# drowe67/radae

Measured on AMD Instinct MI355X. Metric: vocoder-feature frames/sec (enc+chan+dec), model19, higher is better.
Workload: dtype f32 I/O, 2xf16 (22-bit) MFMA operands, f32 accumulate (refine: f64 MFMA)

## Files before the change

radae_amd/csrc/rade_dev.h:

```cpp
#ifndef RADE_DEV_H
#define RADE_DEV_H

#include <stdint.h>

#ifdef __cplusplus
extern "C" {
#endif

#define RD_M        160
#define RD_NCP      32
#define RD_SYM      192
#define RD_NC       30
#define RD_NS       4
#define RD_NMF      960
#define RD_NEOO     1152
#define RD_RXBUF    2112
#define RD_NFC      40
#define RD_NQ       16
#define RD_NTAP     101
#define RD_NINMAX   1120
#define RD_LATENT   80
#define RD_ZMF      240
#define RD_FEAT_MF  432
#define RD_NEOOBITS 180
// ... 61 lines not shown
    int uw_errors, synced_count, snr_int, pad;
    double fmax, Dthresh, Dtmax12, Dtmax12_eoo;
    float snrdB_3k_est; float pad2;
} rd_rx_trace;

typedef void *rd_stream_t;

typedef struct {
    const float *a1; long a1_sb, a1_st; int K1;
    const float *a0; long a0_sb, a0_st; int K0;
    const int *reset; int reset_sb;
    const int *n_rows;
    const float *Wp; const float *bias;
    const unsigned short *Wp16;
    const float *Wscale;
    float *y; long y_sb, y_st; int N;
    int B, T, act;
} rd_gemm_args;
int rd_launch_gemm(const rd_gemm_args *a, rd_stream_t s);
long rd_pack_weights(const float *W, int N, int K, float *out);
long rd_packed_size(int N, int K);

typedef struct {
    const float *gi; long gi_sb, gi_st;
    const float *Whh; const float *bhh;
    float *h;
    float *out; long out_sb, out_st;
    const int *reset; int reset_sb;
    const int *n_rows;
    int B, T, H;
    unsigned short *outf; int outf_NQ, outf_col;
} rd_scan_args;
int rd_launch_gru_scan(const rd_scan_args *a, rd_stream_t s);

#define RD_EF_KB   (RD_ENC_W / 16)
#define RD_EF_TILE (RD_EF_KB * 1024)
typedef struct {
    const unsigned short *xf; int NQ;
    int B, T, K0, K1, dil;
    const unsigned short *Wp16; const float *Wscale; const float *bias; int N, act;
    float *y; long y_sb, y_st;
    unsigned short *yf; int ycol;
    int seq_taps, no_pair;
    int pair;
    const float *xin; int Kin; const float *Wp;
} rd_encf_args;
int rd_launch_encf_gemm(const rd_encf_args *a, rd_stream_t s);
int rd_launch_encf_dense1(const rd_encf_args *a, rd_stream_t s);
int rd_launch_encf_hist(unsigned short *xf, int NQ, float *x32, long x32_sb, int B, int T, int dir, rd_stream_t s);

int rd_launch_enc_pack(const float *features, float *xin, int B, int T, rd_stream_t s);
int rd_launch_pad_rows(const float *src, float *dst, long R, int K, int Kpad, rd_stream_t s);
int rd_launch_chan_symbol(const float *z, const float *H, const float *noise, float *out, long n_real, int mode, float p0, float p1, unsigned long long seed, rd_stream_t s);
int rd_launch_carry_rows(float *x, int B, int Tcap, int W, int nhist, int T, const int *n_rows, rd_stream_t s);
int rd_launch_ofdm_mod(const rd_tables *tab, const float *z, void *tx, long tx_stride, int B, int n_mf, int linear, rd_stream_t s);
int rd_launch_ofdm_mod_mp(const rd_tables *tab, const float *z, void *tx, long tx_stride, int B, int n_mf, const void *G, void *mp, double *part, int linear, rd_stream_t s);
int rd_launch_eoo_build(const rd_tables *tab, const float *bits, float *eoo, int B, rd_stream_t s);
int rd_launch_copy_eoo(const float *eoo, void *out, long stride, int B, rd_stream_t s);

enum { RD_IRX_LS = 0, RD_IRX_MEAN6 = 1, RD_IRX_ALL = 2, RD_IRX_NONE = 3 };
typedef struct {
    const rd_tables *tab; const void *rx; long rx_stride;
    const float *foff;
    int n_mf, time_offset, eq, coarse_mag, B;
    float mag_scale;
    float *z_hat;
// ... 142 lines not shown
```

radae_amd/csrc/rade_devutil.h:

```cpp
#ifndef RADE_DEVUTIL_H
#define RADE_DEVUTIL_H
#include <hip/hip_runtime.h>
#include <stdint.h>
#include <math.h>

#include "rade_dev.h"

typedef float f32x16 __attribute__((ext_vector_type(16)));
typedef float f32x4 __attribute__((ext_vector_type(4)));
typedef float f32x2 __attribute__((ext_vector_type(2)));
typedef unsigned u32x4 __attribute__((ext_vector_type(4)));
__device__ __forceinline__ f32x2 pk_fma(f32x2 a, f32x2 b, f32x2 c) { return __builtin_elementwise_fma(a, b, c); }
typedef double f64x4 __attribute__((ext_vector_type(4)));
typedef _Float16 f16x8 __attribute__((ext_vector_type(8)));

#define PI_D 3.14159265358979323846

__device__ __forceinline__ float2 cmul(float2 a, float2 b) { return make_float2(a.x * b.x - a.y * b.y, a.x * b.y + a.y * b.x); }
__device__ __forceinline__ float2 cmul_nc(float2 a, float2 b)
{
#pragma clang fp contract(off)
    const float rr = a.x * b.x, ii = a.y * b.y, ri = a.x * b.y, ir = a.y * b.x;
    return make_float2(rr - ii, ri + ir);
}
// ... 17 lines not shown
    acc[0] = fmaf(sy.y, -w.y, acc[0]); acc[1] = fmaf(sy.y, w.x, acc[1]);
    return acc;
}

__device__ __forceinline__ float2 cadd(float2 a, float2 b) { return make_float2(a.x + b.x, a.y + b.y); }
__device__ __forceinline__ double chan_phase_acc(int i, float f0, float df_dt)
{
    if (df_dt == 0.0f) { const float om = ((f0 * 2.0f) * (float)PI_D) / 8000.0f; return (double)(i + 1) * (double)om; }
    const double n = (double)(i + 1);
    return (2.0 * PI_D / 8000.0) * (n * (double)f0 + ((double)df_dt / 8000.0) * 0.5 * (double)i * n);
}
__device__ __forceinline__ float2 cconj(float2 a) { return make_float2(a.x, -a.y); }
__device__ __forceinline__ float2 unit_conj(float2 c)
{
    const float n2 = c.x * c.x + c.y * c.y;
    if (n2 == 0.0f) return make_float2(1.0f, 0.0f);
    const float inv = 1.0f / sqrtf(n2);
    return make_float2(c.x * inv, -c.y * inv);
}
__device__ __forceinline__ float2 cis_reduced(double ang)
{
    const double r = ang - 6.283185307179586476925 * rint(ang * 0.15915494309189533577);
    float sn, cs; sincosf((float)r, &sn, &cs);
    return make_float2(cs, sn);
}
__device__ __forceinline__ float sigmoid_f(float x) { return 1.0f / (1.0f + expf(-x)); }
__device__ __forceinline__ int rx_tid() { int t = threadIdx.x; asm volatile("" : "+v"(t)); return t; }
template <int CTRL> __device__ __forceinline__ float quad_dpp(float x) { return __int_as_float(__builtin_amdgcn_update_dpp(0, __float_as_int(x), CTRL, 0xF, 0xF, true)); }
#define QUAD_XOR1 0xB1
#define QUAD_XOR2 0x4E
#define QUAD_BC0  0x00
#define QUAD_BC1  0x55
#define QUAD_BC2  0xAA
#define ROW_ROR4  0x124
#define ROW_ROR8  0x128
template <int CTRL> __device__ __forceinline__ int quad_dpp_i(int x) { return __builtin_amdgcn_update_dpp(0, x, CTRL, 0xF, 0xF, true); }
template <int CTRL> __device__ __forceinline__ double dpp_f64(double x)
{
    const long long b = __double_as_longlong(x);
    const unsigned lo = (unsigned)quad_dpp_i<CTRL>((int)(unsigned)b), hi = (unsigned)quad_dpp_i<CTRL>((int)(unsigned)(b >> 32));
    return __longlong_as_double((long long)(((unsigned long long)hi << 32) | lo));
}
__device__ __forceinline__ double wave_sum_f64(double v)
{
    v += dpp_f64<QUAD_XOR1>(v); v += dpp_f64<QUAD_XOR2>(v); v += dpp_f64<ROW_ROR4>(v); v += dpp_f64<ROW_ROR8>(v);
    const long long b = __double_as_longlong(v);
    double t = 0.0;
#pragma unroll
    for (int r = 0; r < 4; r++) {
        const unsigned lo = (unsigned)__builtin_amdgcn_readlane((int)(unsigned)b, 16 * r), hi = (unsigned)__builtin_amdgcn_readlane((int)(unsigned)(b >> 32), 16 * r);
        t += __longlong_as_double((long long)(((unsigned long long)hi << 32) | lo));
    }
    return t;
}
__device__ __forceinline__ float wave_sum_f32(float v)
{
    v += quad_dpp<QUAD_XOR1>(v); v += quad_dpp<QUAD_XOR2>(v); v += quad_dpp<ROW_ROR4>(v); v += quad_dpp<ROW_ROR8>(v);
    float t = 0.0f;
#pragma unroll
    for (int r = 0; r < 4; r++) t += __int_as_float(__builtin_amdgcn_readlane(__float_as_int(v), 16 * r));
    return t;
}
__device__ __forceinline__ float wave_max_f32(float v)
{
    v = fmaxf(v, quad_dpp<QUAD_XOR1>(v)); v = fmaxf(v, quad_dpp<QUAD_XOR2>(v)); v = fmaxf(v, quad_dpp<ROW_ROR4>(v)); v = fmaxf(v, quad_dpp<ROW_ROR8>(v));
    float t = 0.0f;
// ... 51 lines not shown
```

radae_amd/csrc/rade_engine.c:

```c
#define _GNU_SOURCE
#define __HIP_PLATFORM_AMD__ 1
#include <hip/hip_runtime_api.h>

#include <pthread.h>
#include <time.h>
#include <sched.h>
#include <stdio.h>
#include <stdlib.h>
#include <string.h>
#include <stdint.h>
#include <math.h>

#include "rade_batch.h"
#include "rade_api.h"
#include "rade_host.h"

#define CHK(x) do { hipError_t e_ = (x); if (e_ != hipSuccess) { fprintf(stderr, "rade: HIP error %s at %s:%d\n", hipGetErrorString(e_), __FILE__, __LINE__); goto fail; } } while (0)

static int g_engines_open;
double rade_host_cpu_quota(void)
{
    cpu_set_t set; double n = 1.0;
    if (sched_getaffinity(0, sizeof set, &set) == 0) n = (double)CPU_COUNT(&set);
    FILE *f = fopen("/sys/fs/cgroup/cpu.max", "r");
// ... 9 lines not shown
static pthread_once_t g_sync_once = PTHREAD_ONCE_INIT;
static void sync_policy_init(void)
{
    const char *e = getenv("RADE_SYNC"), *p = getenv("RADE_SYNC_PEERS");
    g_sync_quota = rade_host_cpu_quota(); g_sync_peers = p && atoi(p) > 1 ? atoi(p) : 1;
    g_sync_mode = e && !strcmp(e, "block") ? 1 : (e && !strcmp(e, "spin") ? 0 : 2);
}
static int sync_blocking_now(void)
{
    pthread_once(&g_sync_once, sync_policy_init);
    return g_sync_mode == 2 ? rade_sync_policy(__atomic_load_n(&g_engines_open, __ATOMIC_RELAXED) * g_sync_peers, g_sync_quota) : g_sync_mode;
}

typedef struct { float *wp, *bias; unsigned short *wp16, *wa16; float *wscale, *wscale16; int N, K; } dev_lin;

#define ON_DEV(h) do { if (h) (void)hipSetDevice((h)->device); } while (0)

#define RADE_PROF_MAXEV 256
#define RADE_PROF_MAXIV 4096
struct rade_batch {
    struct owned *owned;
    int alloc_failed;
    int B, max_tx_mf, device, flags, trace_cap, Tcap;
    int R, dec_rows;
    int unsync_off_after;
    unsigned short *corrq16, *corra16, *wfwd16, *bpf16; double *vm; int rx_lds, rx_census;
    int feat_in, enc_kpad, bottleneck1;
    float *dec2_x, *dec2_gi, *dec2_hbuf, *dec2_h[5];
    rd_tables *d_tab;
    dev_lin enc_dense1, enc_zdense, dec_dense1, dec_output, enc_gin[5], dec_gin[5], enc_conv[5], dec_conv[5], dec_glu[5];
    float *enc_whh[5], *enc_bhh[5], *dec_whh[5], *dec_bhh[5];
    unsigned short *dec_whq[5]; float *dec_whs[5];
    float *enc_xin, *enc_x, *enc_gi, *enc_h[5], *enc_z, *eoo, *eoo_bits;
    unsigned short *enc_xf; int enc_nq, enc_seq_taps, enc_no_pair;
    int enc_hist_frag;
    int bypass_dec;
    int tx_linear;
    double *irx_part; long irx_part_cap; float *irx_foff; long long *irx_err;
    rd_bpf_state *tx_bpf, *tx_bpf_init; void *tx_raw; float *tx_chain; float *eoo_filt;
    void *chan_scratch; void *chan_mp;
    float *chan_ps, *chan_ps_host;
    float *rs_sigma; double *rs_part, *rs_stats;
    float *clk_taps; rd_clk_stream *clk_ps, *clk_ps_host;
    int *loss_len; double *loss_res, *loss_part; long loss_part_cap;
    rd_rx_stream *rx_st; rd_rx_round *rx_round;
    int *rx_avail, *rx_acc, *rx_progress, *rx_status;
    float *zrows, *dec_x, *dec_gi, *dec_hbuf, *dec_h[5], *feat84, *dtcache;
    void *rx_filt; float *bpf_chain; long filt_cap, chain_stride;
    rd_rx_trace *trace; float *trace_z;
    long long *wg_cycles;
    int *h_small;
    unsigned *lcg_seeds;
    unsigned *d_lcg_seeds;
    int prof_on, prof_cnt; hipEvent_t prof_ev[2 * RADE_PROF_MAXEV]; int prof_cls[RADE_PROF_MAXEV]; double prof_fl[RADE_PROF_MAXEV];
    double prof_ms[RADE_PROF_NCLASS], prof_flops[RADE_PROF_NCLASS]; long prof_n[RADE_PROF_NCLASS];
    hipEvent_t prof_ref; int iv_n; int iv_cls[RADE_PROF_MAXIV]; float iv_t0[RADE_PROF_MAXIV], iv_t1[RADE_PROF_MAXIV];
    hipEvent_t ev_block;
    long n_sync_block, n_sync_spin;
    double wait_est_us;
};

static const int ENC_IN[5] = { 64, 224, 384, 544, 704 };
static const int ENC_DIL[5] = { 1, 2, 2, 2, 2 };
static const int DEC_IN[5] = { 96, 224, 352, 480, 608 };
static long tx_raw_stride(const rade_batch *h) { return (long)(h->max_tx_mf > 2 ? h->max_tx_mf : 2) * RD_NMF; }

struct owned { struct owned *next; void *p; int pinned; };
// ... 181 lines not shown
    if (h->alloc_failed || h->rx_lds <= 0) goto fail;

    int err = 0;
    h->feat_in = m.enc_dense1.n_in; h->enc_kpad = (h->feat_in + 15) & ~15; h->bottleneck1 = (cfg->flags & RADE_BATCH_BOTTLENECK1) != 0;
    err |= upload_lin(h, &h->enc_dense1, m.enc_dense1.w, m.enc_dense1.b, NULL, 64, h->feat_in, h->enc_kpad);
    err |= upload_lin(h, &h->enc_zdense, m.enc_zdense.w, m.enc_zdense.b, NULL, 80, 864, 864);
    err |= upload_lin(h, &h->dec_dense1, m.dec_dense1.w, m.dec_dense1.b, NULL, 96, 80, 80);
    err |= upload_lin(h, &h->dec_output, m.dec_output.w, m.dec_output.b, NULL, h->feat_in, 736, 736);
    for (int l = 0; l < 5 && !err; l++) {
        err |= upload_lin(h, &h->enc_gin[l], m.enc_gru[l].w_ih, m.enc_gru[l].b_ih, m.enc_gru[l].s_ih, 192, ENC_IN[l], ENC_IN[l]);
        err |= upload_lin(h, &h->dec_gin[l], m.dec_gru[l].w_ih, m.dec_gru[l].b_ih, m.dec_gru[l].s_ih, 288, DEC_IN[l], DEC_IN[l]);
        err |= upload_lin(h, &h->enc_conv[l], m.enc_conv[l].w, m.enc_conv[l].b, m.enc_conv[l].row_scale, 96, m.enc_conv[l].n_in, m.enc_conv[l].n_in);
        err |= upload_lin(h, &h->dec_conv[l], m.dec_conv[l].w, m.dec_conv[l].b, m.dec_conv[l].row_scale, 32, m.dec_conv[l].n_in, m.dec_conv[l].n_in);
        err |= upload_lin(h, &h->dec_glu[l], m.dec_glu[l].w, NULL, m.dec_glu[l].row_scale, 96, 96, 96);
        h->enc_whh[l] = dev_upload(h, m.enc_gru[l].w_hh, sizeof(float) * 192 * 64);
        h->enc_bhh[l] = dev_upload(h, m.enc_gru[l].b_hh, sizeof(float) * 192);
        h->dec_whh[l] = dev_upload(h, m.dec_gru[l].w_hh, sizeof(float) * 288 * 96);
        h->dec_bhh[l] = dev_upload(h, m.dec_gru[l].b_hh, sizeof(float) * 288);
        if (m.dec_gru[l].s_hh) {
            unsigned short *pa = malloc(sizeof(unsigned short) * rd_packed16a_size(288, 96)); float *scl = malloc(sizeof(float) * 288);
            const long nq = (pa && scl) ? rd_pack_weights_q16_a16(m.dec_gru[l].w_hh, m.dec_gru[l].s_hh, 288, 96, pa, scl) : -1;
            if (nq > 0) { h->dec_whq[l] = dev_upload_opt(h, pa, sizeof(unsigned short) * nq); h->dec_whs[l] = dev_upload_opt(h, scl, sizeof(float) * 288); }
            free(pa); free(scl);
        }
    }
    if (err || h->alloc_failed) { fprintf(stderr, "rade: weight upload failed\n"); goto fail; }

    h->enc_xin = dev_zeros(h, sizeof(float) * B * T * RD_ENC_IN);
    h->enc_x = dev_zeros(h, sizeof(float) * B * (2 + T) * RD_ENC_W);
    h->enc_gi = dev_zeros(h, sizeof(float) * B * T * 192);
    h->enc_nq = 1 + (h->Tcap + 31) / 32;
    h->enc_seq_taps = getenv("RADE_ENCF_SEQ_TAPS") != NULL;
    h->enc_no_pair = getenv("RADE_ENCF_NO_PAIR") != NULL;
    if (B * T > 16384 && !getenv("RADE_ENC_ROWS")) {
        h->enc_xf = dev_alloc_opt(h, sizeof(unsigned short) * B * h->enc_nq * RD_EF_TILE, 1);
        if (!h->enc_xf && !getenv("RADE_VERBOSE_0"))
            fprintf(stderr, "rade: no device memory for the encoder's fragment buffer (%.1f MB): the float32-row kernels serve every call (slower encoder GEMMs, same results to the last bits documented in rade_batch.h)\n",
                    1e-6 * sizeof(unsigned short) * (double)B * h->enc_nq * RD_EF_TILE);
    }
    h->enc_z = dev_zeros(h, sizeof(float) * B * T * RD_LATENT);
    h->eoo = dev_zeros(h, sizeof(float) * B * RD_NEOO * 2);
    h->eoo_bits = dev_zeros(h, sizeof(float) * B * RD_NEOOBITS);
    h->bypass_dec = (cfg->flags & RADE_BATCH_BYPASS_DEC) != 0;
    h->tx_linear = (cfg->flags & RADE_BATCH_TX_LINEAR) != 0;
    if (h->tx_linear && (cfg->flags & RADE_BATCH_TX_BPF)) { fprintf(stderr, "rade: RADE_BATCH_TX_LINEAR cannot be combined with RADE_BATCH_TX_BPF (the filter clips)\n"); goto fail; }
    if (cfg->flags & RADE_BATCH_TX_BPF) {
        rd_bpf_state *init = calloc(B, sizeof *init);
        if (!init) goto fail;
        for (size_t b = 0; b < B; b++) { init[b].mem_len = 100; init[b].phase[0] = 1.0f; }
        h->tx_bpf_init = dev_upload(h, init, sizeof(rd_bpf_state) * B); h->tx_bpf = dev_upload(h, init, sizeof(rd_bpf_state) * B);
        free(init);
        h->tx_raw = dev_zeros(h, sizeof(float) * 2 * B * tx_raw_stride(h));
        h->tx_chain = dev_zeros(h, sizeof(float) * 2 * B * (cfg->max_tx_mf + 8));
        h->eoo_filt = dev_zeros(h, sizeof(float) * 2 * B * RD_NEOO);
    }
    h->chan_scratch = dev_zeros(h, sizeof(double) * B * (1 + (cfg->max_tx_mf > 64 ? cfg->max_tx_mf : 64)) * 2);
    h->enc_h[0] = dev_zeros(h, sizeof(float) * 5 * B * 64); h->dec_h[0] = dev_zeros(h, sizeof(float) * 5 * B * 96);
    h->dec2_h[0] = dev_zeros(h, sizeof(float) * 5 * B * 96);
    h->rx_progress = dev_zeros(h, sizeof(int) * (8 + B * 8));
    if (h->alloc_failed) { fprintf(stderr, "rade: device allocation failed\n"); goto fail; }
    for (int l = 1; l < 5; l++) { h->enc_h[l] = h->enc_h[0] + (size_t)l * B * 64; h->dec_h[l] = h->dec_h[0] + (size_t)l * B * 96; }
    for (int l = 1; l < 5; l++) h->dec2_h[l] = h->dec2_h[0] + (size_t)l * B * 96;
    h->rx_acc = h->rx_progress + 8; h->rx_status = h->rx_progress + 8 + 4 * B;
    h->rx_st = dev_zeros(h, sizeof(rd_rx_stream) * B);
    h->rx_round = dev_zeros(h, sizeof(rd_rx_round) * B);
    h->rx_avail = dev_zeros(h, sizeof(int) * B);
// ... 116 lines not shown
    PROF_END(hh, stream, RADE_PROF_GEMM, 2.0 * (double)B * T * (K0 + K1) * w->N);
    return rc;
}

static int encf_gemm(rade_batch *h, const dev_lin *w, int K1, int K0, int dil, float *y, long y_sb, long y_st, int ycol, int T, int act, void *stream)
{
    rd_encf_args g;
    memset(&g, 0, sizeof g);
    g.xf = h->enc_xf; g.NQ = h->enc_nq; g.B = h->B; g.T = T; g.K0 = K0; g.K1 = K1; g.dil = dil;
    g.Wp16 = w->wp16; g.Wscale = w->wscale16; g.bias = w->bias; g.N = w->N; g.act = act;
    g.y = y; g.y_sb = y_sb; g.y_st = y_st; if (!y) { g.yf = h->enc_xf; g.ycol = ycol; }
    g.seq_taps = h->enc_seq_taps; g.no_pair = h->enc_no_pair;
    if (K0 + K1 != w->K || !w->wp16) { fprintf(stderr, "rade: internal GEMM shape error (%d+%d != %d)\n", K0, K1, w->K); return -1; }
    PROF_BEGIN(h, stream);
    const int rc = rd_launch_encf_gemm(&g, stream);
    PROF_END(h, stream, RADE_PROF_GEMM, 2.0 * (double)h->B * T * (K0 + K1) * w->N);
    return rc;
}
static int encode_core_frag(rade_batch *h, int T, float *z, void *stream)
{
    const int B = h->B;
    int e = h->enc_hist_frag ? 0 : rd_launch_encf_hist(h->enc_xf, h->enc_nq, h->enc_x, (long)(2 + h->Tcap) * RD_ENC_W, B, T, 0, stream);
    {
        rd_encf_args g;
        memset(&g, 0, sizeof g);
        g.xf = h->enc_xf; g.NQ = h->enc_nq; g.B = B; g.T = T; g.bias = h->enc_dense1.bias; g.N = 64; g.act = 1; g.yf = h->enc_xf; g.ycol = 0;
        g.xin = h->enc_xin; g.Kin = h->enc_kpad; g.Wp = h->enc_dense1.wp;
        PROF_BEGIN(h, stream); e |= rd_launch_encf_dense1(&g, stream); PROF_END(h, stream, RADE_PROF_GEMM, 2.0 * (double)B * T * h->enc_kpad * 64);
    }
    e |= encf_gemm(h, &h->enc_gin[0], ENC_IN[0], 0, 0, h->enc_gi, (long)T * 192, 192, 0, T, 0, stream);
    for (int l = 0; l < 5 && !e; l++) {
        const int in = ENC_IN[l], cin = in + 64;
        rd_scan_args s = { h->enc_gi, (long)T * 192, 192, h->enc_whh[l], h->enc_bhh[l], h->enc_h[l], NULL, 0, 0, NULL, 0, NULL, B, T, 64, h->enc_xf, h->enc_nq, in };
        PROF_BEGIN(h, stream); e |= rd_launch_gru_scan(&s, stream); PROF_END(h, stream, RADE_PROF_SCAN, 2.0 * B * T * 192 * 64);
        e |= encf_gemm(h, &h->enc_conv[l], cin, cin, ENC_DIL[l], NULL, 0, 0, cin, T, 1, stream);
        if (l < 4) e |= encf_gemm(h, &h->enc_gin[l + 1], ENC_IN[l + 1], 0, 0, h->enc_gi, (long)T * 192, 192, 0, T, 0, stream);
        else e |= encf_gemm(h, &h->enc_zdense, 864, 0, 0, z, (long)T * RD_LATENT, RD_LATENT, 0, T, h->bottleneck1 ? 1 : 0, stream);
    }
    e |= rd_launch_encf_hist(h->enc_xf, h->enc_nq, h->enc_x, (long)(2 + h->Tcap) * RD_ENC_W, B, T, 1, stream);
    h->enc_hist_frag = !e;
    return e;
}

static int encode_core(rade_batch *h, int T, float *z, void *stream)
{
    const int B = h->B, W = RD_ENC_W;
    if (h->enc_xf && (long)B * T > 16384) return encode_core_frag(h, T, z, stream);
    h->enc_hist_frag = 0;
    const long xsb = (long)(2 + h->Tcap) * W;
    float *x0 = h->enc_x + 2 * W;
    int e = 0;
    dev_lin d1 = h->enc_dense1; d1.wp16 = NULL; d1.wscale16 = NULL;
    e |= gemm(h, &d1, h->enc_xin, (long)T * h->enc_kpad, h->enc_kpad, h->enc_kpad, NULL, 0, 0, 0, NULL, NULL, x0, xsb, W, B, T, 1, stream);
    for (int l = 0; l < 5 && !e; l++) {
        const int in = ENC_IN[l], cin = in + 64;
        e |= gemm(h, &h->enc_gin[l], x0, xsb, W, in, NULL, 0, 0, 0, NULL, NULL, h->enc_gi, (long)T * 192, 192, B, T, 0, stream);
        rd_scan_args s = { h->enc_gi, (long)T * 192, 192, h->enc_whh[l], h->enc_bhh[l], h->enc_h[l], x0 + in, xsb, W, NULL, 0, NULL, B, T, 64 };
        PROF_BEGIN(h, stream); e |= rd_launch_gru_scan(&s, stream); PROF_END(h, stream, RADE_PROF_SCAN, 2.0 * B * T * 192 * 64);
        e |= gemm(h, &h->enc_conv[l], x0, xsb, W, cin, x0 - (long)ENC_DIL[l] * W, xsb, W, cin, NULL, NULL, x0 + cin, xsb, W, B, T, 1, stream);
    }
    e |= gemm(h, &h->enc_zdense, x0, xsb, W, 864, NULL, 0, 0, 0, NULL, NULL, z, (long)T * RD_LATENT, RD_LATENT, B, T, h->bottleneck1 ? 1 : 0, stream);
    e |= rd_launch_carry_rows(h->enc_x, B, h->Tcap, W, 2, T, NULL, stream);
    return e;
}

static int tx_bpf_pass(rade_batch *h, int n, int len0, void *out, long out_stride, void *stream, int advance)
{
    rd_bpf_args ba;
    memset(&ba, 0, sizeof ba);
    ba.state = h->tx_bpf; ba.state_stride = sizeof(rd_bpf_state); ba.len0_const = len0; ba.avail_const = n;
    ba.tab = h->d_tab; ba.bpf16 = h->bpf16; ba.x = h->tx_raw; ba.x_stride = tx_raw_stride(h); ba.y = out; ba.y_stride = out_stride;
    ba.chain = h->tx_chain; ba.chain_stride = h->max_tx_mf + 8; ba.n_blocks = 1 + (n > len0 ? (n - len0 + RD_NMF - 1) / RD_NMF : 0); ba.B = h->B; ba.clip = 1; ba.advance = advance;
    PROF_BEGIN(h, stream);
    const int rc = rd_launch_bpf(&ba, stream);
    PROF_END(h, stream, RADE_PROF_BPF, 8.0 * 101.0 * (double)h->B * n);
    return rc;
}

static int encode_features(rade_batch *h, const float *features_dev, int T, float *z, void *stream)
{
    const int e = rd_launch_enc_pack(features_dev, h->enc_xin, h->B, T, stream);
    return e | encode_core(h, T, z, stream);
}
static int modulate(rade_batch *h, const float *z, int n_mf, void *iq_out, long iq_stride, void *stream)
{
    void *mod_out = h->tx_bpf ? h->tx_raw : iq_out; const long mod_stride = h->tx_bpf ? tx_raw_stride(h) : iq_stride;
    PROF_BEGIN(h, stream);
    int e = rd_launch_ofdm_mod(h->d_tab, z, mod_out, mod_stride, h->B, n_mf, h->tx_linear, stream);
    PROF_END(h, stream, RADE_PROF_MOD, 8.0 * h->B * n_mf * 5 * 30 * 160);
    if (h->tx_bpf) e |= tx_bpf_pass(h, n_mf * RD_NMF, RD_NMF, iq_out, iq_stride, stream, 1);
    return e;
// ... 164 lines not shown
    if (hipMalloc((void **)&taps, sizeof(float) * n_taps) != hipSuccess || hipMemcpy(taps, fir_taps_host, sizeof(float) * n_taps, hipMemcpyHostToDevice) != hipSuccess) { hipFree(taps); return -1; }
    void *ybuf = NULL;
    if (rd_multipath_gen_needs_scratch(low_ratio, n_out)) {
        const size_t n_low = (size_t)(n_out + low_ratio - 1) / low_ratio;
        if (hipMalloc(&ybuf, sizeof(double) * 2 * 2 * n_low * h->B) != hipSuccess) { hipFree(taps); return -1; }
    }
    const int rc = rd_launch_multipath_gen(taps, n_taps, low_ratio, n_out, noise_low_dev, seed, G_out_dev, ybuf, h->B, stream);
    hipStreamSynchronize((hipStream_t)stream);
    hipFree(taps);
    if (ybuf) hipFree(ybuf);
    return rc ? -1 : n_out;
}

int rade_batch_multipath_h(rade_batch *h, const void *G_dev, int n_g, int fs_over_rs, int n_sym, int Nc, float delay_s, float Rs, int want_complex, float *H_out_dev, void *stream)
{
    ON_DEV(h);
    if (!h || !G_dev || !H_out_dev) return -1;
    return rd_launch_multipath_h(G_dev, n_g, fs_over_rs, n_sym, Nc, delay_s * Rs, want_complex, H_out_dev, h->B, stream) ? -1 : n_sym;
}

static int decoder_layers(rade_batch *h, const float *z, int T, int Tio, int Tcap, float *xbuf, float *gi, float *hbuf, float **hstate,
                          const int *nr, const int *rst, float *out, void *stream)
{
    const int B = h->B, W = RD_DEC_W;
    const long xsb = (long)(1 + Tcap) * W;
    float *x = xbuf + W;
    int e = 0;
    dev_lin d1 = h->dec_dense1; d1.wp16 = NULL; d1.wscale16 = NULL;
    e |= gemm(h, &d1, z, (long)Tio * RD_LATENT, RD_LATENT, RD_LATENT, NULL, 0, 0, 0, NULL, nr, x, xsb, W, B, T, 1, stream);
    for (int l = 0; l < 5 && !e; l++) {
        const int in = DEC_IN[l];
        e |= gemm(h, &h->dec_gin[l], x, xsb, W, in, NULL, 0, 0, 0, NULL, nr, gi, (long)T * 288, 288, B, T, 0, stream);
        rd_scan_args s = { gi, (long)T * 288, 288, h->dec_whh[l], h->dec_bhh[l], hstate[l], hbuf, (long)T * 96, 96, rst, h->dec_rows, nr, B, T, 96 };
        PROF_BEGIN(h, stream); e |= rd_launch_gru_scan(&s, stream); PROF_END(h, stream, RADE_PROF_SCAN, 2.0 * B * T * 288 * 96);
        e |= gemm(h, &h->dec_glu[l], hbuf, (long)T * 96, 96, 96, NULL, 0, 0, 0, NULL, nr, x + in, xsb, W, B, T, 2, stream);
        const int cin = in + 96;
        e |= gemm(h, &h->dec_conv[l], x, xsb, W, cin, x - W, xsb, W, cin, rst, nr, x + cin, xsb, W, B, T, 1, stream);
    }
    e |= gemm(h, &h->dec_output, x, xsb, W, 736, NULL, 0, 0, 0, NULL, nr, out, (long)Tio * h->feat_in, h->feat_in, B, T, 0, stream);
    return e;
}

static void fill_dec_args(const rade_batch *h, rd_decs_args *d)
{
    memset(d, 0, sizeof *d);
    const long DR = h->dec_rows;
    d->z = h->zrows; d->z_sb = DR * RD_LATENT; d->x = h->dec_x + RD_DEC_W; d->x_sb = (1 + DR) * RD_DEC_W;
    d->gi = h->dec_gi; d->gi_sb = DR * 288; d->hbuf = h->dec_hbuf; d->hb_sb = DR * 96;
    d->out = h->feat84; d->out_sb = DR * h->feat_in; d->out_w = h->feat_in;
    d->B = h->B;
#define LIN(dst, src) do { (dst).wp = (src).wp; (dst).bias = (src).bias; (dst).wp16 = (src).wp16; (dst).wa16 = (src).wa16; (dst).wscale = (src).wscale; (dst).N = (src).N; (dst).K = (src).K; } while (0)
    LIN(d->dense1, h->dec_dense1); LIN(d->output, h->dec_output);
    for (int l = 0; l < 5; l++) { LIN(d->gin[l], h->dec_gin[l]); LIN(d->glu[l], h->dec_glu[l]); LIN(d->conv[l], h->dec_conv[l]); d->whh[l] = h->dec_whh[l]; d->bhh[l] = h->dec_bhh[l]; d->h[l] = h->dec_h[l];
                                  d->whq[l] = (h->dec_whq[l] && h->dec_whs[l]) ? h->dec_whq[l] : NULL; d->whs[l] = h->dec_whs[l]; }
#undef LIN
}

int rade_batch_decode(rade_batch *h, const float *z_dev, int n_steps, float *features_out_dev, int reset_state, void *stream)
{
    ON_DEV(h);
    if (!h || !z_dev || n_steps <= 0 || n_steps > h->Tcap || !features_out_dev) return -1;
    if (misaligned16(z_dev)) return -1;
    hipStream_t st = (hipStream_t)stream;
    if (reset_state) {
        hipMemsetAsync(h->dec2_h[0], 0, sizeof(float) * 5 * h->B * 96, st);
        hipMemsetAsync(h->dec2_x, 0, sizeof(float) * (size_t)h->B * (1 + h->Tcap) * RD_DEC_W, st);
    }
// ... 283 lines not shown
```

radae_amd/csrc/rade_kernels.hip:

```cpp
#include "rade_devutil.h"

__device__ float g_zero_row[2048];

template <int NT>
__global__ __launch_bounds__(64) void k_gemm(rd_gemm_args a)
{
    const int lane = threadIdx.x;
    const int rows = a.B * a.T;
    const int r0 = blockIdx.x * 32;
    const int ntt = (a.N + 31) >> 5;
    const int nt0 = blockIdx.y * NT;
    int r = r0 + (lane & 31);
    if (r >= rows) r = rows - 1;
    const int b = r / a.T, t = r - b * a.T;
    const int half = lane >> 5;
    const float *p1 = a.a1 + b * a.a1_sb + t * a.a1_st + 4 * half;
    const float *p0 = nullptr;
    if (a.K0) {
        const bool rst = a.reset && a.reset[b * a.reset_sb + t];
        p0 = (rst ? g_zero_row : a.a0 + b * a.a0_sb + t * a.a0_st) + 4 * half;
    }
    f32x16 acc[NT];
#pragma unroll
    for (int i = 0; i < NT; i++)
// ... 337 lines not shown
        int &attr_done = attr_done_dev[dev_ & 63];
        if (!attr_done) {
            (void)hipFuncSetAttribute((const void *)k_gemm_splitk<3>, hipFuncAttributeMaxDynamicSharedMemorySize, SK_WAVES * 3 * 16 * 64 * 4);
            (void)hipFuncSetAttribute((const void *)k_gemm_splitk<2>, hipFuncAttributeMaxDynamicSharedMemorySize, SK_WAVES * 2 * 16 * 64 * 4);
            (void)hipFuncSetAttribute((const void *)k_gemm_splitk<1>, hipFuncAttributeMaxDynamicSharedMemorySize, SK_WAVES * 1 * 16 * 64 * 4);
            attr_done = 1;
        }
        if (ntt % 3 == 0) hipLaunchKernelGGL(k_gemm_splitk<3>, dim3(gx, ntt / 3), block, SK_WAVES * 3 * 16 * 64 * 4, st, *a);
        else if (ntt % 2 == 0) hipLaunchKernelGGL(k_gemm_splitk<2>, dim3(gx, ntt / 2), block, SK_WAVES * 2 * 16 * 64 * 4, st, *a);
        else hipLaunchKernelGGL(k_gemm_splitk<1>, dim3(gx, ntt), block, SK_WAVES * 1 * 16 * 64 * 4, st, *a);
        return (int)hipGetLastError();
    }
    dim3 block(64);
    if (a->Wp16 && (a->K0 & 15) == 0 && (a->K1 & 15) == 0) {
        const int gx2 = (rows + 63) / 64;
        if ((((a->K0 + a->K1) >> 4) & 1) == 0 && ((a->K0 >> 4) & 1) == 0 && ntt % 3 == 0) {
            if (a->Wscale) { dim3 g1(gx, ntt / 3); hipLaunchKernelGGL((k_gemm16p<3, 1, true>), g1, block, 0, st, *a); return (int)hipGetLastError(); }
            dim3 grid(gx2, ntt / 3);
            hipLaunchKernelGGL((k_gemm16p<3, 2, false>), grid, block, 0, st, *a);
            return (int)hipGetLastError();
        }
        if (ntt % 3 == 0) { dim3 grid(gx2, ntt / 3); hipLaunchKernelGGL((k_gemm16<3, 2>), grid, block, 0, st, *a); }
        else if (ntt % 2 == 0) { dim3 grid(gx2, ntt / 2); hipLaunchKernelGGL((k_gemm16<2, 2>), grid, block, 0, st, *a); }
        else { dim3 grid(gx2, ntt); hipLaunchKernelGGL((k_gemm16<1, 2>), grid, block, 0, st, *a); }
        return (int)hipGetLastError();
    }
    if (ntt % 3 == 0) { dim3 grid(gx, ntt / 3); hipLaunchKernelGGL(k_gemm<3>, grid, block, 0, st, *a); }
    else if (ntt % 2 == 0) { dim3 grid(gx, ntt / 2); hipLaunchKernelGGL(k_gemm<2>, grid, block, 0, st, *a); }
    else { dim3 grid(gx, ntt); hipLaunchKernelGGL(k_gemm<1>, grid, block, 0, st, *a); }
    return (int)hipGetLastError();
}

template <int H>
__global__ __launch_bounds__(4 * H) void k_gru_scan(rd_scan_args a)
{
    __builtin_amdgcn_s_setprio(3);
    constexpr int KP = H / 4;
    __shared__ __attribute__((aligned(16))) float hs[2][H];
    __shared__ int rst[RD_DEC_ROWS_MAX];
    const int b = blockIdx.x, tid = threadIdx.x, j = tid >> 2, p = tid & 3;
    float wr[KP], wz[KP], wn[KP];
    {
        const float *w0 = a.Whh + (size_t)j * H + p * KP;
#pragma unroll
        for (int k = 0; k < KP; k += 4) {
            const f32x4 v0 = *(const f32x4 *)(w0 + k), v1 = *(const f32x4 *)(w0 + (size_t)H * H + k), v2 = *(const f32x4 *)(w0 + (size_t)2 * H * H + k);
#pragma unroll
            for (int u = 0; u < 4; u++) { wr[k + u] = v0[u]; wz[k + u] = v1[u]; wn[k + u] = v2[u]; }
        }
    }
    const float br = a.bhh[j], bz = a.bhh[H + j], bn = a.bhh[2 * H + j];
    const int Tb = a.n_rows ? a.n_rows[b] : a.T;
    if (a.reset) for (int i = tid; i < a.T && i < RD_DEC_ROWS_MAX; i += blockDim.x) rst[i] = a.reset[b * a.reset_sb + i];
    float hj = a.h[(size_t)b * H + j];
    if (p == 0) hs[0][j] = hj;
    _Float16 *of = nullptr;
    if (a.outf) { const int col = a.outf_col + j; of = (_Float16 *)a.outf + (size_t)b * a.outf_NQ * RD_EF_TILE + (col >> 4) * 1024 + ((col >> 3) & 1) * 256 + (col & 7); }
    const float *gi = a.gi + (size_t)b * a.gi_sb + (p < 3 ? p * H + j : j);
    float gA[4], gB[4];
    auto fetch = [&](float (&dst)[4], int t0) {
#pragma unroll
        for (int u = 0; u < 4; u++) dst[u] = gi[(size_t)min(t0 + u, max(Tb - 1, 0)) * a.gi_st];
    };
    __builtin_amdgcn_s_waitcnt(0x0F70);
    __builtin_amdgcn_sched_barrier(0);
    fetch(gA, 0); fetch(gB, 4);
    __syncthreads();
// ... 25 lines not shown
                const f32x2 h0 = { hv[0], hv[1] }, h1 = { hv[2], hv[3] };
                ar = __builtin_elementwise_fma((f32x2){ wr[k], wr[k + 1] }, h0, ar); az = __builtin_elementwise_fma((f32x2){ wz[k], wz[k + 1] }, h0, az); an = __builtin_elementwise_fma((f32x2){ wn[k], wn[k + 1] }, h0, an);
                ar = __builtin_elementwise_fma((f32x2){ wr[k + 2], wr[k + 3] }, h1, ar); az = __builtin_elementwise_fma((f32x2){ wz[k + 2], wz[k + 3] }, h1, az); an = __builtin_elementwise_fma((f32x2){ wn[k + 2], wn[k + 3] }, h1, an);
            }
            if (of && tpend >= 0) store_frag(tpend);
            float sr = ar[0] + ar[1], sz = az[0] + az[1], sn = an[0] + an[1];
            sr += quad_dpp<QUAD_XOR1>(sr); sz += quad_dpp<QUAD_XOR1>(sz); sn += quad_dpp<QUAD_XOR1>(sn);
            sr += quad_dpp<QUAD_XOR2>(sr); sz += quad_dpp<QUAD_XOR2>(sz); sn += quad_dpp<QUAD_XOR2>(sn);
            const float g0 = gq[u];
            const float gr = quad_dpp<QUAD_BC0>(g0), gz = quad_dpp<QUAD_BC1>(g0), gn = quad_dpp<QUAD_BC2>(g0);
            const float r = gate_sigmoid((sr + br) + gr);
            const float z = gate_sigmoid((sz + bz) + gz);
            const float n = gate_tanh(gn + (sn + bn) * r);
            hj = (hj - n) * z + n;
            if (p == 0) {
                hs[cur ^ 1][j] = hj;
                if (!of) a.out[(size_t)b * a.out_sb + (size_t)t * a.out_st + j] = clamp1(hj);
            }
            pend = hj; tpend = t;
            cur ^= 1;
            __syncthreads();
        }
    };
    for (int t0 = 0; t0 < Tb; t0 += 8) {
        block(gA, t0);
        fetch(gA, t0 + 8);
        block(gB, t0 + 4);
        fetch(gB, t0 + 12);
    }
    if (of && tpend >= 0) store_frag(tpend);
    if (p == 0) a.h[(size_t)b * H + j] = hj;
}

extern "C" int rd_launch_gru_scan(const rd_scan_args *a, rd_stream_t s)
{
    if (a->B <= 0) return 0;
    hipStream_t st = (hipStream_t)s;
    if (a->H == 64) hipLaunchKernelGGL(k_gru_scan<64>, dim3(a->B), dim3(256), 0, st, *a);
    else if (a->H == 96) hipLaunchKernelGGL(k_gru_scan<96>, dim3(a->B), dim3(384), 0, st, *a);
    else return -1;
    return (int)hipGetLastError();
}

__global__ void k_enc_pack(const float *features, float *xin, int B, int T)
{
    __builtin_amdgcn_s_setprio(3);
    const long n = (long)B * T * RD_ENC_IN;
    for (long i = blockIdx.x * (long)blockDim.x + threadIdx.x; i < n; i += (long)gridDim.x * blockDim.x) {
        const int c = (int)(i % RD_ENC_IN); const long bt = i / RD_ENC_IN;
        float v = 0.0f;
        if (c < 84) { const int fr = c / 21, j = c - fr * 21; v = j < 20 ? features[(bt * 4 + fr) * 36 + j] : -1.0f; }
        xin[i] = v;
    }
}
extern "C" int rd_launch_enc_pack(const float *features, float *xin, int B, int T, rd_stream_t s)
{
    const long n = (long)B * T * RD_ENC_IN; if (n <= 0) return 0;
    int grid = (int)((n + 255) / 256); if (grid > 4096) grid = 4096;
    hipLaunchKernelGGL(k_enc_pack, dim3(grid), dim3(256), 0, (hipStream_t)s, features, xin, B, T);
    return (int)hipGetLastError();
}

__global__ void k_pad_rows(const float *src, float *dst, long R, int K, int Kpad)
{
    const long n = R * Kpad;
    for (long i = blockIdx.x * (long)blockDim.x + threadIdx.x; i < n; i += (long)gridDim.x * blockDim.x) {
        const int c = (int)(i % Kpad); const long r = i / Kpad;
        dst[i] = c < K ? src[r * K + c] : 0.0f;
    }
}
extern "C" int rd_launch_pad_rows(const float *src, float *dst, long R, int K, int Kpad, rd_stream_t s)
{
    const long n = R * Kpad; if (n <= 0) return 0;
    int grid = (int)((n + 255) / 256); if (grid > 4096) grid = 4096;
    hipLaunchKernelGGL(k_pad_rows, dim3(grid), dim3(256), 0, (hipStream_t)s, src, dst, R, K, Kpad);
// ... 397 lines not shown
```

Baseline: 86.87 million.

## Add 2-lane-per-unit GRU scan kernel and make it the default

Adds a GRU recurrent scan variant that splits each hidden unit's dot product across 2 threads instead of 4, so each thread holds twice the weights and does twice the FMAs per step. Blocks shrink to 2*H threads, and gate inputs are distributed with quad DPP even/odd broadcasts. The goal is fewer cross-lane reduction steps, fewer waves per block, and cheaper barriers on the serial time loop, at the cost of longer per-thread FMA chains and higher register pressure. The old 4-lane kernel stays selectable through RADE_SCAN_LANES=4.

```diff
diff --git a/radae_amd/csrc/rade_dev.h b/radae_amd/csrc/rade_dev.h
--- a/radae_amd/csrc/rade_dev.h
+++ b/radae_amd/csrc/rade_dev.h
@@ -117,6 +117,7 @@
     unsigned short *outf; int outf_NQ, outf_col;
 } rd_scan_args;
 int rd_launch_gru_scan(const rd_scan_args *a, rd_stream_t s);
+int rd_launch_gru_scan_lanes(const rd_scan_args *a, int lanes, rd_stream_t s);
 
 #define RD_EF_KB   (RD_ENC_W / 16)
 #define RD_EF_TILE (RD_EF_KB * 1024)
diff --git a/radae_amd/csrc/rade_devutil.h b/radae_amd/csrc/rade_devutil.h
--- a/radae_amd/csrc/rade_devutil.h
+++ b/radae_amd/csrc/rade_devutil.h
@@ -73,6 +73,8 @@
 #define QUAD_BC0  0x00
 #define QUAD_BC1  0x55
 #define QUAD_BC2  0xAA
+#define QUAD_EVEN 0xA0
+#define QUAD_ODD  0xF5
 #define ROW_ROR4  0x124
 #define ROW_ROR8  0x128
 template <int CTRL> __device__ __forceinline__ int quad_dpp_i(int x) { return __builtin_amdgcn_update_dpp(0, x, CTRL, 0xF, 0xF, true); }
diff --git a/radae_amd/csrc/rade_engine.c b/radae_amd/csrc/rade_engine.c
--- a/radae_amd/csrc/rade_engine.c
+++ b/radae_amd/csrc/rade_engine.c
@@ -65,7 +65,7 @@
     float *enc_whh[5], *enc_bhh[5], *dec_whh[5], *dec_bhh[5];
     unsigned short *dec_whq[5]; float *dec_whs[5];
     float *enc_xin, *enc_x, *enc_gi, *enc_h[5], *enc_z, *eoo, *eoo_bits;
-    unsigned short *enc_xf; int enc_nq, enc_seq_taps, enc_no_pair;
+    unsigned short *enc_xf; int enc_nq, enc_seq_taps, enc_no_pair, scan_lanes;
     int enc_hist_frag;
     int bypass_dec;
     int tx_linear;
@@ -313,6 +313,7 @@
     h->enc_nq = 1 + (h->Tcap + 31) / 32;
     h->enc_seq_taps = getenv("RADE_ENCF_SEQ_TAPS") != NULL;
     h->enc_no_pair = getenv("RADE_ENCF_NO_PAIR") != NULL;
+    { const char *sl = getenv("RADE_SCAN_LANES"); h->scan_lanes = (sl && atoi(sl) == 4) ? 4 : 2; }
     if (B * T > 16384 && !getenv("RADE_ENC_ROWS")) {
         h->enc_xf = dev_alloc_opt(h, sizeof(unsigned short) * B * h->enc_nq * RD_EF_TILE, 1);
         if (!h->enc_xf && !getenv("RADE_VERBOSE_0"))
@@ -495,7 +496,7 @@
     for (int l = 0; l < 5 && !e; l++) {
         const int in = ENC_IN[l], cin = in + 64;
         rd_scan_args s = { h->enc_gi, (long)T * 192, 192, h->enc_whh[l], h->enc_bhh[l], h->enc_h[l], NULL, 0, 0, NULL, 0, NULL, B, T, 64, h->enc_xf, h->enc_nq, in };
-        PROF_BEGIN(h, stream); e |= rd_launch_gru_scan(&s, stream); PROF_END(h, stream, RADE_PROF_SCAN, 2.0 * B * T * 192 * 64);
+        PROF_BEGIN(h, stream); e |= rd_launch_gru_scan_lanes(&s, h->scan_lanes, stream); PROF_END(h, stream, RADE_PROF_SCAN, 2.0 * B * T * 192 * 64);
         e |= encf_gemm(h, &h->enc_conv[l], cin, cin, ENC_DIL[l], NULL, 0, 0, cin, T, 1, stream);
         if (l < 4) e |= encf_gemm(h, &h->enc_gin[l + 1], ENC_IN[l + 1], 0, 0, h->enc_gi, (long)T * 192, 192, 0, T, 0, stream);
         else e |= encf_gemm(h, &h->enc_zdense, 864, 0, 0, z, (long)T * RD_LATENT, RD_LATENT, 0, T, h->bottleneck1 ? 1 : 0, stream);
@@ -519,7 +520,7 @@
         const int in = ENC_IN[l], cin = in + 64;
         e |= gemm(h, &h->enc_gin[l], x0, xsb, W, in, NULL, 0, 0, 0, NULL, NULL, h->enc_gi, (long)T * 192, 192, B, T, 0, stream);
         rd_scan_args s = { h->enc_gi, (long)T * 192, 192, h->enc_whh[l], h->enc_bhh[l], h->enc_h[l], x0 + in, xsb, W, NULL, 0, NULL, B, T, 64 };
-        PROF_BEGIN(h, stream); e |= rd_launch_gru_scan(&s, stream); PROF_END(h, stream, RADE_PROF_SCAN, 2.0 * B * T * 192 * 64);
+        PROF_BEGIN(h, stream); e |= rd_launch_gru_scan_lanes(&s, h->scan_lanes, stream); PROF_END(h, stream, RADE_PROF_SCAN, 2.0 * B * T * 192 * 64);
         e |= gemm(h, &h->enc_conv[l], x0, xsb, W, cin, x0 - (long)ENC_DIL[l] * W, xsb, W, cin, NULL, NULL, x0 + cin, xsb, W, B, T, 1, stream);
     }
     e |= gemm(h, &h->enc_zdense, x0, xsb, W, 864, NULL, 0, 0, 0, NULL, NULL, z, (long)T * RD_LATENT, RD_LATENT, B, T, h->bottleneck1 ? 1 : 0, stream);
@@ -750,7 +751,7 @@
         const int in = DEC_IN[l];
         e |= gemm(h, &h->dec_gin[l], x, xsb, W, in, NULL, 0, 0, 0, NULL, nr, gi, (long)T * 288, 288, B, T, 0, stream);
         rd_scan_args s = { gi, (long)T * 288, 288, h->dec_whh[l], h->dec_bhh[l], hstate[l], hbuf, (long)T * 96, 96, rst, h->dec_rows, nr, B, T, 96 };
-        PROF_BEGIN(h, stream); e |= rd_launch_gru_scan(&s, stream); PROF_END(h, stream, RADE_PROF_SCAN, 2.0 * B * T * 288 * 96);
+        PROF_BEGIN(h, stream); e |= rd_launch_gru_scan_lanes(&s, h->scan_lanes, stream); PROF_END(h, stream, RADE_PROF_SCAN, 2.0 * B * T * 288 * 96);
         e |= gemm(h, &h->dec_glu[l], hbuf, (long)T * 96, 96, 96, NULL, 0, 0, 0, NULL, nr, x + in, xsb, W, B, T, 2, stream);
         const int cin = in + 96;
         e |= gemm(h, &h->dec_conv[l], x, xsb, W, cin, x - W, xsb, W, cin, rst, nr, x + cin, xsb, W, B, T, 1, stream);
diff --git a/radae_amd/csrc/rade_kernels.hip b/radae_amd/csrc/rade_kernels.hip
--- a/radae_amd/csrc/rade_kernels.hip
+++ b/radae_amd/csrc/rade_kernels.hip
@@ -393,7 +393,7 @@
 }
 
 template <int H>
-__global__ __launch_bounds__(4 * H) void k_gru_scan(rd_scan_args a)
+__global__ __launch_bounds__(4 * H) void k_gru_scan4(rd_scan_args a)
 {
     __builtin_amdgcn_s_setprio(3);
     constexpr int KP = H / 4;
@@ -485,15 +485,110 @@
     if (p == 0) a.h[(size_t)b * H + j] = hj;
 }
 
-extern "C" int rd_launch_gru_scan(const rd_scan_args *a, rd_stream_t s)
+template <int H>
+__global__ __launch_bounds__(2 * H) void k_gru_scan(rd_scan_args a)
+{
+    __builtin_amdgcn_s_setprio(3);
+    constexpr int KP = H / 4;
+    __shared__ __attribute__((aligned(16))) float hs[2][H];
+    __shared__ int rst[RD_DEC_ROWS_MAX];
+    const int b = blockIdx.x, tid = threadIdx.x, j = tid >> 1, p = tid & 1;
+    float wr[2 * KP], wz[2 * KP], wn[2 * KP];
+    {
+        const float *w0 = a.Whh + (size_t)j * H + p * 2 * KP;
+#pragma unroll
+        for (int k = 0; k < 2 * KP; k += 4) {
+            const f32x4 v0 = *(const f32x4 *)(w0 + k), v1 = *(const f32x4 *)(w0 + (size_t)H * H + k), v2 = *(const f32x4 *)(w0 + (size_t)2 * H * H + k);
+#pragma unroll
+            for (int u = 0; u < 4; u++) { wr[k + u] = v0[u]; wz[k + u] = v1[u]; wn[k + u] = v2[u]; }
+        }
+    }
+    const float br = a.bhh[j], bz = a.bhh[H + j], bn = a.bhh[2 * H + j];
+    const int Tb = a.n_rows ? a.n_rows[b] : a.T;
+    if (a.reset) for (int i = tid; i < a.T && i < RD_DEC_ROWS_MAX; i += blockDim.x) rst[i] = a.reset[b * a.reset_sb + i];
+    float hj = a.h[(size_t)b * H + j];
+    if (p == 0) hs[0][j] = hj;
+    _Float16 *of = nullptr;
+    if (a.outf) { const int col = a.outf_col + j; of = (_Float16 *)a.outf + (size_t)b * a.outf_NQ * RD_EF_TILE + (col >> 4) * 1024 + ((col >> 3) & 1) * 256 + (col & 7) + p * 512; }
+    const float *gi = a.gi + (size_t)b * a.gi_sb + p * H + j, *gin = a.gi + (size_t)b * a.gi_sb + 2 * H + j;
+    float gA[4], gB[4], nA[4], nB[4];
+    auto fetch = [&](float (&dst)[4], float (&dstn)[4], int t0) {
+#pragma unroll
+        for (int u = 0; u < 4; u++) { const size_t o = (size_t)min(t0 + u, max(Tb - 1, 0)) * a.gi_st; dst[u] = gi[o]; dstn[u] = gin[o]; }
+    };
+    __builtin_amdgcn_s_waitcnt(0x0F70);
+    __builtin_amdgcn_sched_barrier(0);
+    fetch(gA, nA, 0); fetch(gB, nB, 4);
+    __syncthreads();
+    int cur = 0;
+    float pend = 0.0f; int tpend = -1;
+    auto store_frag = [&](int tp) {
+        const float x = 256.0f * clamp1(pend); const _Float16 hi = (_Float16)x, lo = (_Float16)(x - (float)hi);
+        of[(size_t)(1 + (tp >> 5)) * RD_EF_TILE + (tp & 31) * 8] = p ? lo : hi;
+    };
+    auto block = [&](const float (&gq)[4], const float (&gnq)[4], int t0) {
+#pragma unroll
+        for (int u = 0; u < 4; u++) {
+            const int t = t0 + u;
+            if (t >= Tb) break;
+            if (a.reset && rst[t]) {
+                hj = 0.0f;
+                __syncthreads();
+                if (p == 0) hs[cur][j] = 0.0f;
+                __syncthreads();
+            }
+            f32x2 ar0 = { 0.0f, 0.0f }, az0 = ar0, an0 = ar0, ar1 = ar0, az1 = ar0, an1 = ar0;
+            const float *hp = hs[cur] + p * 2 * KP;
+#pragma unroll
+            for (int k = 0; k < KP; k += 4) {
+                const f32x4 hv = *(const f32x4 *)(hp + k), hw = *(const f32x4 *)(hp + KP + k);
+                const f32x2 h0 = { hv[0], hv[1] }, h1 = { hv[2], hv[3] }, h2 = { hw[0], hw[1] }, h3 = { hw[2], hw[3] };
+                ar0 = __builtin_elementwise_fma((f32x2){ wr[k], wr[k + 1] }, h0, ar0); az0 = __builtin_elementwise_fma((f32x2){ wz[k], wz[k + 1] }, h0, az0); an0 = __builtin_elementwise_fma((f32x2){ wn[k], wn[k + 1] }, h0, an0);
+                ar1 = __builtin_elementwise_fma((f32x2){ wr[KP + k], wr[KP + k + 1] }, h2, ar1); az1 = __builtin_elementwise_fma((f32x2){ wz[KP + k], wz[KP + k + 1] }, h2, az1); an1 = __builtin_elementwise_fma((f32x2){ wn[KP + k], wn[KP + k + 1] }, h2, an1);
+                ar0 = __builtin_elementwise_fma((f32x2){ wr[k + 2], wr[k + 3] }, h1, ar0); az0 = __builtin_elementwise_fma((f32x2){ wz[k + 2], wz[k + 3] }, h1, az0); an0 = __builtin_elementwise_fma((f32x2){ wn[k + 2], wn[k + 3] }, h1, an0);
+                ar1 = __builtin_elementwise_fma((f32x2){ wr[KP + k + 2], wr[KP + k + 3] }, h3, ar1); az1 = __builtin_elementwise_fma((f32x2){ wz[KP + k + 2], wz[KP + k + 3] }, h3, az1); an1 = __builtin_elementwise_fma((f32x2){ wn[KP + k + 2], wn[KP + k + 3] }, h3, an1);
+            }
+            if (of && tpend >= 0) store_frag(tpend);
+            float sr = (ar0[0] + ar0[1]) + (ar1[0] + ar1[1]), sz = (az0[0] + az0[1]) + (az1[0] + az1[1]), sn = (an0[0] + an0[1]) + (an1[0] + an1[1]);
+            sr += quad_dpp<QUAD_XOR1>(sr); sz += quad_dpp<QUAD_XOR1>(sz); sn += quad_dpp<QUAD_XOR1>(sn);
+            const float g0 = gq[u];
+            const float gr = quad_dpp<QUAD_EVEN>(g0), gz = quad_dpp<QUAD_ODD>(g0), gn = gnq[u];
+            const float r = gate_sigmoid((sr + br) + gr);
+            const float z = gate_sigmoid((sz + bz) + gz);
+            const float n = gate_tanh(gn + (sn + bn) * r);
+            hj = (hj - n) * z + n;
+            if (p == 0) {
+                hs[cur ^ 1][j] = hj;
+                if (!of) a.out[(size_t)b * a.out_sb + (size_t)t * a.out_st + j] = clamp1(hj);
+            }
+            pend = hj; tpend = t;
+            cur ^= 1;
+            __syncthreads();
+        }
+    };
+    for (int t0 = 0; t0 < Tb; t0 += 8) {
+        block(gA, nA, t0);
+        fetch(gA, nA, t0 + 8);
+        block(gB, nB, t0 + 4);
+        fetch(gB, nB, t0 + 12);
+    }
+    if (of && tpend >= 0) store_frag(tpend);
+    if (p == 0) a.h[(size_t)b * H + j] = hj;
+}
+
+extern "C" int rd_launch_gru_scan_lanes(const rd_scan_args *a, int lanes, rd_stream_t s)
 {
     if (a->B <= 0) return 0;
     hipStream_t st = (hipStream_t)s;
-    if (a->H == 64) hipLaunchKernelGGL(k_gru_scan<64>, dim3(a->B), dim3(256), 0, st, *a);
-    else if (a->H == 96) hipLaunchKernelGGL(k_gru_scan<96>, dim3(a->B), dim3(384), 0, st, *a);
+    if (lanes == 2 && a->H == 64) hipLaunchKernelGGL(k_gru_scan<64>, dim3(a->B), dim3(128), 0, st, *a);
+    else if (lanes == 2 && a->H == 96) hipLaunchKernelGGL(k_gru_scan<96>, dim3(a->B), dim3(192), 0, st, *a);
+    else if (lanes == 4 && a->H == 64) hipLaunchKernelGGL(k_gru_scan4<64>, dim3(a->B), dim3(256), 0, st, *a);
+    else if (lanes == 4 && a->H == 96) hipLaunchKernelGGL(k_gru_scan4<96>, dim3(a->B), dim3(384), 0, st, *a);
     else return -1;
     return (int)hipGetLastError();
 }
+
+extern "C" int rd_launch_gru_scan(const rd_scan_args *a, rd_stream_t s) { return rd_launch_gru_scan_lanes(a, 2, s); }
 
 __global__ void k_enc_pack(const float *features, float *xin, int B, int T)
 {
```

New measurement: 82.42 million. 5.1% lower.
